# RC4ML/Legion

Hardware: AMD Instinct MI355X
Metric: sampled_edges_per_sec (higher is better)
Workload: dtype int32+f32(copy)

## Files before the change

### legion_amd/csrc/kernels_gather.hip

```cpp
#include "legion_core.h"
#include "gather_plan.h"

#include <cstdlib>
#include <cstring>
#include <type_traits>

namespace lg {

#define LG_GATHER_THREADS 256

__device__ __forceinline__ void deliver_slice(const LanePtrs& L, const DeliverParams& d, int32_t part, int32_t parts)
{
    const LG_G int32_t* nc = LG_GPTR(const int32_t, L.node_counter);
    const LG_G int32_t* ec = LG_GPTR(const int32_t, L.edge_counter);
    const LG_G int32_t* hs = LG_GPTR(const int32_t, L.hop_scratch);
    const int32_t hop_num = nc[INTRABATCH_CON * 3 - 1];
    int32_t n = nc[INTRABATCH_CON * 3 + hop_num], e = ec[INTRABATCH_CON * 3 + hop_num], b = nc[INTRABATCH_CON * 3];
    n = n < 0 ? 0 : (n > d.num_ids ? d.num_ids : n);
    e = e < 0 ? 0 : (e > d.num_ids ? d.num_ids : e);
    b = b < 0 ? 0 : (b > d.batch_cap ? d.batch_cap : b);
    const int32_t tid = threadIdx.x, nthr = blockDim.x;
    typedef int32_t v4 __attribute__((ext_vector_type(4)));
    auto copy = [&](const int32_t* src, int32_t* dst, int32_t count) {
        const int32_t per = (((count + parts - 1) / parts) + 3) & ~3;
        const int32_t lo = part * per, hi = min(lo + per, count);
        if (lo >= hi) return;
        const LG_G v4* s4 = (const LG_G v4*)(src + lo);
        LG_G v4* d4 = (LG_G v4*)(dst + lo);
        const int32_t q = (hi - lo) >> 2;
        for (int32_t i = tid; i < q; i += nthr) d4[i] = s4[i];
        for (int32_t i = lo + (q << 2) + tid; i < hi; i += nthr) LG_GPTR(int32_t, dst)[i] = LG_GPTR(const int32_t, src)[i];
    };
    copy(L.sampled_ids, d.sampled_ids, n);
    copy(L.agg_src_off, d.agg_src_off, e);
    copy(L.agg_dst_off, d.agg_dst_off, e);
    copy(L.labels, d.labels, b);
    if (part == 0 && tid < 32) {
        int32_t v = tid < 16 ? nc[tid] : ec[tid - 16];
        if (tid == 2) v = hs[HS_RANGE + 2 * hop_num];
        if (tid == 3) v = hs[HS_RANGE + 2 * hop_num + 1];
        LG_GPTR(int32_t, tid < 16 ? d.node_counter : d.edge_counter)[tid & 15] = v;
        if (d.mirror != nullptr) LG_GPTR(int32_t, d.mirror)[tid] = v;
    }
}

__global__ __launch_bounds__(256) void deliver_kernel(const LanePtrs* __restrict__ lane_p, DeliverParams d)
{
    deliver_slice(*lane_p, d, blockIdx.x, gridDim.x);
}

void launch_deliver(hipStream_t s, const LanePtrs* d_lane, const DeliverParams& d)
{
    int32_t grid = (d.num_ids / 4 + 1023) / 1024;
    if (grid > 512) grid = 512;
    if (grid < 1) grid = 1;
    deliver_kernel<<<grid, 256, 0, s>>>(d_lane, d);
    hipCheckError();
}

typedef float f32x4 __attribute__((ext_vector_type(4)));
template <typename VecT, bool TAIL> struct GatherRow {
    static_assert(std::is_same<VecT, f32x4>::value || std::is_same<VecT, float>::value, "float32 rows; bf16 rows have no TAIL pass");
    typedef float Out;
    static __device__ int32_t chunks(const GatherParams& gp) { return gp.D / (int32_t)(sizeof(VecT) / sizeof(float)); }
    static __device__ const LG_G float* row_at(const GatherParams& gp, const float* base, int64_t x) { return LG_GPTR(const float, base) + x * gp.D; }
    static __device__ VecT load(const LG_G float* p, bool, LG_G float* dst_tile, int32_t r, int32_t c, int32_t D)
    {
        if (p == nullptr) p = dst_tile + (int64_t)r * D;
        return ((const LG_G VecT*)p)[c];
    }
    static __device__ void store(const VecT& v, bool ok, LG_G float* dst_tile, int32_t r, int32_t c, int32_t D)
    {
        if (ok) __builtin_nontemporal_store(v, (LG_G VecT*)(dst_tile + (int64_t)r * D) + c);
    }
};

struct Bf16x8 {
    typedef uint32_t u4 __attribute__((ext_vector_type(4)));
    u4 w;
};
struct Bf16Copy : Bf16x8 {};
__device__ __attribute__((aligned(16))) Bf16x8 lg_gather_zero_line;
template <typename VecT, typename OutT> struct GatherRowBf16Src {
    typedef OutT Out;
    static __device__ int32_t chunks(const GatherParams& gp) { return gp.pitch / 8; }
    static __device__ const LG_G float* row_at(const GatherParams& gp, const float* base, int64_t x)
    {
        return (const LG_G float*)(LG_GPTR(const uint16_t, (const uint16_t*)base) + x * gp.pitch);
    }
    static __device__ VecT load(const LG_G float* p, bool has, LG_G Out*, int32_t, int32_t c, int32_t)
    {
        VecT v;
        v.w = has ? ((const LG_G VecT*)p)[c].w : LG_GPTR(const Bf16x8, &lg_gather_zero_line)->w;
        return v;
    }
};

template <> struct GatherRow<Bf16x8, false> : GatherRowBf16Src<Bf16x8, float> {
    static __device__ void store(const Bf16x8& v, bool ok, LG_G float* dst_tile, int32_t r, int32_t c, int32_t D)
    {
        typedef float v4u __attribute__((ext_vector_type(4), aligned(4)));
        typedef Bf16x8::u4 u4;
        const u4 lo = v.w << 16, hi = v.w & 0xFFFF0000u;
        const int32_t e0 = c * 8;
        LG_G float* d = dst_tile + (int64_t)r * D + e0;
        if (ok && e0 + 8 <= D) {
            __builtin_nontemporal_store(__builtin_bit_cast(v4u, u4{lo.x, hi.x, lo.y, hi.y}), (LG_G v4u*)d);
            __builtin_nontemporal_store(__builtin_bit_cast(v4u, u4{lo.z, hi.z, lo.w, hi.w}), (LG_G v4u*)d + 1);
        } else if (ok) {
            const uint32_t f[8] = {lo.x, hi.x, lo.y, hi.y, lo.z, hi.z, lo.w, hi.w};
#pragma unroll
            for (int k = 0; k < 8; k++)
                if (e0 + k < D) d[k] = __uint_as_float(f[k]);
        }
    }
};

__device__ __forceinline__ void gather_store_bf16(const uint32_t (&w)[4], bool ok, LG_G uint16_t* dst_tile, int32_t r, int32_t c, int32_t D)
{
    typedef uint32_t u4u __attribute__((ext_vector_type(4), aligned(4)));
    const int32_t e0 = c * 8;
    LG_G uint16_t* d = dst_tile + (int64_t)r * D + e0;
    if (ok && (D & 1) == 0) {
        if (e0 + 8 <= D) {
            __builtin_nontemporal_store(u4u{w[0], w[1], w[2], w[3]}, (LG_G u4u*)d);
        } else {
#pragma unroll
            for (int k = 0; k < 4; k++)
                if (e0 + 2 * k < D) ((LG_G uint32_t*)d)[k] = w[k];
        }
    } else if (ok) {
#pragma unroll
        for (int k = 0; k < 8; k++)
            if (e0 + k < D) d[k] = (uint16_t)(w[k >> 1] >> ((k & 1) * 16));
    }
}

template <> struct GatherRow<Bf16Copy, false> : GatherRowBf16Src<Bf16Copy, uint16_t> {
    static __device__ void store(const Bf16Copy& v, bool ok, LG_G uint16_t* dst_tile, int32_t r, int32_t c, int32_t D)
    {
        gather_store_bf16({v.w.x, v.w.y, v.w.z, v.w.w}, ok, dst_tile, r, c, D);
    }
};
__device__ __forceinline__ uint32_t gather_bf16_rne(float f)
{
    const uint32_t u = __float_as_uint(f);
    if ((u & 0x7FFFFFFFu) > 0x7F800000u) return (u >> 16) | 0x40u;
    return (u + 0x7FFFu + ((u >> 16) & 1u)) >> 16;
}

struct F32Narrow {
    typedef float v4u __attribute__((ext_vector_type(4), aligned(4)));
    v4u a, b;
};
template <> struct GatherRow<F32Narrow, false> {
    typedef uint16_t Out;
    typedef F32Narrow::v4u v4u;
    static __device__ int32_t chunks(const GatherParams& gp) { return (gp.D + 7) / 8; }
    static __device__ const LG_G float* row_at(const GatherParams& gp, const float* base, int64_t x) { return LG_GPTR(const float, base) + x * gp.D; }
    static __device__ F32Narrow load(const LG_G float* p, bool, LG_G uint16_t*, int32_t, int32_t c, int32_t D)
    {
        F32Narrow v;
        const int32_t e0 = c * 8;
        if (p == nullptr) {
            v.a = v.b = v4u{0.f, 0.f, 0.f, 0.f};
        } else if (e0 + 8 <= D) {
            v.a = ((const LG_G v4u*)(p + e0))[0];
            v.b = ((const LG_G v4u*)(p + e0))[1];
        } else {
            float f[8];
#pragma unroll
            for (int k = 0; k < 8; k++) f[k] = e0 + k < D ? p[e0 + k] : 0.f;
            v.a = v4u{f[0], f[1], f[2], f[3]};
            v.b = v4u{f[4], f[5], f[6], f[7]};
        }
        return v;
    }
    static __device__ void store(const F32Narrow& v, bool ok, LG_G uint16_t* dst_tile, int32_t r, int32_t c, int32_t D)
    {
        gather_store_bf16({gather_bf16_rne(v.a.x) | (gather_bf16_rne(v.a.y) << 16), gather_bf16_rne(v.a.z) | (gather_bf16_rne(v.a.w) << 16),
                           gather_bf16_rne(v.b.x) | (gather_bf16_rne(v.b.y) << 16), gather_bf16_rne(v.b.z) | (gather_bf16_rne(v.b.w) << 16)},
                          ok, dst_tile, r, c, D);
    }
};

#ifndef LG_GATHER_MIN_WAVES
#define LG_GATHER_MIN_WAVES 8
#endif
#ifndef LG_GATHER_TARGET_WG
#define LG_GATHER_TARGET_WG 8192
#endif

template <typename VecT, int ROWS, int UNROLL, bool TAIL, bool LASTOP>
__global__ __launch_bounds__(LG_GATHER_THREADS, LG_GATHER_MIN_WAVES) void gather_kernel(GatherParams gp, const LanePtrs* __restrict__ lanes,
                                                                   bool copy_range)
{
    typedef GatherRow<VecT, TAIL> Row;
    typedef typename Row::Out Out;
    constexpr int VEC = sizeof(VecT) / sizeof(float);
    static_assert(ROWS <= LG_GATHER_THREADS, "one resolving thread per row of a tile");
    __shared__ const LG_G float* s_ptr[2][ROWS];

    const LanePtrs& L = lanes[blockIdx.y];
    const LG_G int32_t* range = LG_GPTR(const int32_t, gp.hop >= 0 ? L.hop_scratch + HS_RANGE + 2 * gp.hop : L.node_counter);
    const LG_G int32_t* sampled_ids = LG_GPTR(const int32_t, L.sampled_ids);
    const LG_G int32_t* node_slot = (L.node_slot != nullptr && gp.node_map != nullptr) ? LG_GPTR(const int32_t, L.node_slot) : nullptr;
    LG_G int32_t* cache_search_buffer = LG_GPTR(int32_t, L.cache_search_buffer);
    int32_t off = range[0];
    int32_t rows = range[1];
    if (copy_range && blockIdx.x == 0 && threadIdx.x == 0) {
        LG_GPTR(int32_t, L.node_counter)[2] = off;
        LG_GPTR(int32_t, L.node_counter)[3] = rows;
    }
    if (gp.hop >= 0 && gp.first_hop < gp.hop) {
        const int32_t off0 = LG_GPTR(const int32_t, L.hop_scratch)[HS_RANGE + 2 * gp.first_hop];
        rows += off - off0;
        off = off0;
    }
    if (rows > gp.max_rows) rows = gp.max_rows;
    if (rows > L.feature_rows - off) {
        rows = L.feature_rows - off;
        if (blockIdx.x == 0 && threadIdx.x == 0 && L.hop_scratch != nullptr) {
            __hip_atomic_fetch_or(LG_GPTR(int32_t, L.hop_scratch) + HS_ERROR, LG_ERR_FEATURE_ROWS, __ATOMIC_RELAXED, __HIP_MEMORY_SCOPE_AGENT);
            if (L.err_flag) __hip_atomic_fetch_or(LG_GPTR(int32_t, L.err_flag), LG_ERR_FEATURE_ROWS, __ATOMIC_RELAXED, __HIP_MEMORY_SCOPE_SYSTEM);
        }
    }
    const int32_t ntiles = (rows + ROWS - 1) / ROWS;
    const int32_t step = gridDim.x;
    if (LASTOP && L.deliver != nullptr)
        deliver_slice(L, *static_cast<const DeliverParams*>(L.deliver), blockIdx.x, step);
    const int32_t tid = threadIdx.x;
    const int32_t D = gp.D;
    const int32_t C = Row::chunks(gp);
    const int32_t dr = LG_GATHER_THREADS / C;
    const int32_t dc = LG_GATHER_THREADS - dr * C;
    int32_t tile = blockIdx.x;
    if (tile >= ntiles) return;

    const bool counting = gp.stats != nullptr && gp.Kg > 1 && gp.stats[3] != 0ull;
    auto source_of = [&](int32_t id, int32_t g) -> const LG_G float* {
        const LG_G float* p = nullptr;
        if (g < 0) {
            if (id >= 0 && gp.full_table != nullptr)
                p = Row::row_at(gp, gp.full_table, (int64_t)(id < gp.total_num_nodes ? id : id % gp.total_num_nodes));
        } else if (gp.hybrid) {
            if (g < gp.hybrid_cpu_cap)
                p = Row::row_at(gp, gp.hybrid_cpu_cache, (int64_t)g);
            else
                p = Row::row_at(gp, gp.local_table, (int64_t)((g - gp.hybrid_cpu_cap) % gp.hybrid_gpu_cap));
        } else {
            int32_t didx = 0, fidx = g;
            if (gp.striped) { didx = g / gp.node_capacity; fidx = g - didx * gp.node_capacity; }
            const int64_t rank = (int64_t)fidx * gp.Kg + didx;
            const bool local_copy = gp.replica != nullptr && rank < gp.replica_rows;
            if (local_copy)
                p = Row::row_at(gp, gp.replica, rank);
            else if (didx == gp.member && gp.local_table != nullptr)
                p = Row::row_at(gp, gp.local_table, (int64_t)fidx);
            else if (gp.skip_remote)
                p = nullptr;
            else
                p = Row::row_at(gp, gp.cache_tables[didx], (int64_t)fidx);
            if (counting) {
                const unsigned long long m_rep = __ballot(local_copy), m_str = __ballot(!local_copy);
                const unsigned long long m_peer = __ballot(!local_copy && didx != gp.member);
                if ((int)(threadIdx.x & 63) == __ffsll((unsigned long long)(m_rep | m_str)) - 1) {
                    if (m_str) atomicAdd(gp.stats + 0, (unsigned long long)__popcll(m_str));
                    if (m_rep) atomicAdd(gp.stats + 1, (unsigned long long)__popcll(m_rep));
                    if (m_peer) atomicAdd(gp.stats + 2, (unsigned long long)__popcll(m_peer));
                }
            }
        }
        return p;
    };
    auto lookup = [&](int32_t id, int32_t carried) -> int32_t {
        if (carried != LG_FS_UNKNOWN) return carried;
        return (gp.node_map != nullptr && id >= 0) ? gp.node_map[id] : CACHEMISS_FLAG;
    };

    int32_t id_n = -1, fs_n = LG_FS_UNKNOWN;
    bool have_n = false;
    if (tid < ROWS) {
        const int32_t r = tile * ROWS + tid;
        if (r < rows) {
            const int32_t id = sampled_ids[off + r];
            const int32_t g = lookup(id, node_slot != nullptr ? node_slot[off + r] : LG_FS_UNKNOWN);
            cache_search_buffer[r] = g;
            s_ptr[0][tid] = source_of(id, g);
        }
        const int32_t rn = (tile + step) * ROWS + tid;
        have_n = tile + step < ntiles && rn < rows;
        if (have_n) {
            id_n = sampled_ids[off + rn];
            if (node_slot != nullptr) fs_n = node_slot[off + rn];
        }
    }
    __syncthreads();

    int buf = 0;
    for (; tile < ntiles; tile += step) {
        const int32_t r0 = tile * ROWS;
        const int32_t nr = min(ROWS, rows - r0);
        int32_t g_n = CACHEMISS_FLAG, id_nn = -1, fs_nn = LG_FS_UNKNOWN;
        bool have_nn = false;
        if (tid < ROWS) {
            if (have_n) g_n = lookup(id_n, fs_n);
            const int32_t rnn = (tile + 2 * step) * ROWS + tid;
            have_nn = tile + 2 * step < ntiles && rnn < rows;
            if (have_nn) {
                id_nn = sampled_ids[off + rnn];
                if (node_slot != nullptr) fs_nn = node_slot[off + rnn];
            }
        }

        const int32_t nchunks = nr * C;
        LG_G Out* dst_tile = LG_GPTR(Out, (Out*)L.float_features) + (int64_t)(off + r0) * D;
        int32_t q = tid;
        int32_t r = q / C;
        int32_t c = q - r * C;
        while (q < nchunks) {
            VecT v[UNROLL];
            int32_t rr[UNROLL], cc[UNROLL];
            bool ok[UNROLL];
#pragma unroll
            for (int u = 0; u < UNROLL; u++) {
                const bool in = q < nchunks;
                rr[u] = in ? r : nr - 1;
                cc[u] = in ? c : C - 1;
                const LG_G float* p = s_ptr[buf][rr[u]];
                ok[u] = in && p != nullptr;
                v[u] = Row::load(p, p != nullptr, dst_tile, rr[u], cc[u], D);
                q += LG_GATHER_THREADS;
                r += dr;
                c += dc;
                if (c >= C) { c -= C; r += 1; }
            }
#pragma unroll
            for (int u = 0; u < UNROLL; u++) Row::store(v[u], ok[u], dst_tile, rr[u], cc[u], D);
        }
        if constexpr (TAIL) {
            const int32_t tail = D - C * VEC;
            for (int32_t i = tid; i < nr * tail; i += LG_GATHER_THREADS) {
                const int32_t tr = i / tail, k = C * VEC + (i - tr * tail);
                const LG_G float* p = s_ptr[buf][tr];
                if (p != nullptr) dst_tile[(int64_t)tr * D + k] = p[k];
            }
        }
        if (tid < ROWS && have_n) {
            cache_search_buffer[(tile + step) * ROWS + tid] = g_n;
            s_ptr[buf ^ 1][tid] = source_of(id_n, g_n);
        }
        id_n = id_nn;
        fs_n = fs_nn;
        have_n = have_nn;
        __syncthreads();
        buf ^= 1;
    }
}

__global__ __launch_bounds__(256) void bulk_bucket_kernel(GatherParams gp, const LanePtrs* __restrict__ lanes, BulkLists b, const char* arena_base)
{
    const LanePtrs& L = lanes[blockIdx.y];
    const LG_G int32_t* nc = LG_GPTR(const int32_t, L.node_counter);
    const int32_t hop_num = nc[INTRABATCH_CON * 3 - 1];
    int32_t n = nc[INTRABATCH_CON * 3 + hop_num];
    if (n > L.feature_rows) n = L.feature_rows;
    if (n > gp.max_rows) n = gp.max_rows;
    const LG_G int32_t* sampled_ids = LG_GPTR(const int32_t, L.sampled_ids);
    const LG_G int32_t* node_slot = (L.node_slot != nullptr && gp.node_map != nullptr) ? LG_GPTR(const int32_t, L.node_slot) : nullptr;
    const int32_t lane = threadIdx.x & 63;
    for (int32_t r0 = (blockIdx.x * 256 + (threadIdx.x & ~63)); r0 < n; r0 += gridDim.x * 256) {
        const int32_t r = r0 + lane;
        int32_t owner = -1, fidx = 0;
        if (r < n) {
            const int32_t id = sampled_ids[r];
            int32_t g = node_slot != nullptr ? node_slot[r] : LG_FS_UNKNOWN;
            if (g == LG_FS_UNKNOWN) g = (gp.node_map != nullptr && id >= 0) ? gp.node_map[id] : CACHEMISS_FLAG;
            if (g >= 0) {
                const int32_t didx = g / gp.node_capacity;
                fidx = g - didx * gp.node_capacity;
                const int64_t rank = (int64_t)fidx * gp.Kg + didx;
                const bool local_copy = gp.replica != nullptr && rank < gp.replica_rows;
                if (!local_copy && didx != gp.member) owner = didx;
            }
        }
        for (int32_t o = 0; o < b.Kg; o++) {
            const unsigned long long m = __ballot(owner == o);
            if (m == 0ull) continue;
            unsigned long long base = 0;
            if (lane == __ffsll((long long)m) - 1) base = atomicAdd(b.cnt + o, (unsigned long long)__popcll(m));
            base = __shfl(base, __ffsll((long long)m) - 1);
            if (owner == o) {
                const int64_t at = (int64_t)base + __popcll(m & ((lane == 0) ? 0ull : (~0ull >> (64 - lane))));
                if (at < b.cap) {
                    b.fidx[(int64_t)o * b.cap + at] = fidx;
                    b.dst[(int64_t)o * b.cap + at] = (const char*)(L.float_features + (int64_t)r * gp.D) - arena_base;
                }
            }
        }
    }
}

void launch_bulk_bucket(hipStream_t s, const GatherParams& g, const LanePtrs* d_lanes, int32_t n_lanes, const BulkLists& lists,
                        const char* arena_base)
{
    if (g.D <= 0 || g.max_rows <= 0 || g.node_map == nullptr || g.Kg <= 1) return;
    GatherParams gp = g;
    if (gp.node_capacity < 1) gp.node_capacity = 1;
    int32_t gx = (g.max_rows + 255) / 256;
    while (gx > 16 && (int64_t)gx * n_lanes > 16384) gx = (gx + 1) / 2;
    bulk_bucket_kernel<<<dim3(gx, n_lanes), 256, 0, s>>>(gp, d_lanes, lists, arena_base);
    hipCheckError();
}

__global__ __launch_bounds__(256) void bulk_push_kernel(const float* __restrict__ stripe, int32_t D, const int32_t* __restrict__ fidx,
                                                       const int64_t* __restrict__ dst, const unsigned long long* __restrict__ cnt,
                                                       int64_t cap, char* __restrict__ peer_arena)
{
    typedef float v4u __attribute__((ext_vector_type(4), aligned(4)));
    int64_t n = (int64_t)cnt[0];
    if (n > cap) n = cap;
    const int32_t lane = threadIdx.x & 63;
    const int64_t wave = ((int64_t)blockIdx.x * 256 + threadIdx.x) >> 6, nwaves = ((int64_t)gridDim.x * 256) >> 6;
    const int32_t C = D / 4;
    for (int64_t i = wave; i < n; i += nwaves) {
        const LG_G float* src = LG_GPTR(const float, stripe) + (int64_t)fidx[i] * D;
        LG_G float* out = (LG_G float*)(peer_arena + dst[i]);
        for (int32_t c = lane; c < C; c += 64) ((LG_G v4u*)out)[c] = ((const LG_G v4u*)src)[c];
        for (int32_t k = C * 4 + lane; k < D; k += 64) out[k] = src[k];
    }
}

void launch_bulk_push(hipStream_t s, const float* stripe, int32_t D, const int32_t* fidx, const int64_t* dst,
                      const unsigned long long* cnt, int64_t cap, char* peer_arena)
{
    if (stripe == nullptr || D <= 0 || cap <= 0) return;
    bulk_push_kernel<<<2048, 256, 0, s>>>(stripe, D, fidx, dst, cnt, cap, peer_arena);
    hipCheckError();
}

static inline int32_t gather_grid_x(int32_t max_rows, int32_t rows_per_tile, int32_t n_lanes)
{
    const int32_t tiles = (max_rows + rows_per_tile - 1) / rows_per_tile;
    int32_t gx = (LG_GATHER_TARGET_WG + n_lanes - 1) / n_lanes;
    if (gx > tiles) gx = tiles;
    return gx < 1 ? 1 : gx;
}

template <typename VecT, GatherFormat F, int ROWS = 16>
static int32_t launch_format(hipStream_t s, int32_t rows, const GatherParams& gk, int32_t grid_rows, const LanePtrs* d_lanes, int32_t n_lanes, bool copy_range)
{
    constexpr GatherFormatInfo fi = gather_info(F);
    if constexpr ((fi.tiles & ROWS) != 0) {
        if (rows == ROWS) {
            const dim3 grid(gather_grid_x(grid_rows, ROWS, n_lanes), n_lanes);
            if (gk.last_op) gather_kernel<VecT, ROWS, fi.unroll, fi.tail, true><<<grid, LG_GATHER_THREADS, 0, s>>>(gk, d_lanes, copy_range);
            else gather_kernel<VecT, ROWS, fi.unroll, fi.tail, false><<<grid, LG_GATHER_THREADS, 0, s>>>(gk, d_lanes, copy_range);
            return (int32_t)grid.x;
        }
    }
    if constexpr (ROWS < 256) return launch_format<VecT, F, ROWS * 2>(s, rows, gk, grid_rows, d_lanes, n_lanes, copy_range);
    return 0;
}

static GatherPlan plan_of_launch(const GatherParams& gk, int32_t n_lanes, int32_t& grid_rows)
{
    grid_rows = gk.grid_rows > 0 && gk.grid_rows < gk.max_rows ? gk.grid_rows : gk.max_rows;
    return gather_plan(gk.dtype, gk.out_dtype, gk.D, gk.pitch, grid_rows, n_lanes, tuning().gather_rows_per_wg);
}

static GatherPlan launch_gather_impl(hipStream_t s, GatherParams gk, const LanePtrs* d_lanes, int32_t n_lanes, bool copy_range, int32_t* grid_x = nullptr)
{
    if (grid_x != nullptr) *grid_x = 0;
    if (gk.D <= 0 || gk.max_rows <= 0) return {GatherPlan::OK, GatherFormat::F32, 0};
    if (gk.node_capacity < 1) gk.node_capacity = 1;
    int32_t grid_rows, gx = 0;
    const GatherPlan p = plan_of_launch(gk, n_lanes, grid_rows);
    if (p.error == GatherPlan::BAD_DTYPE) printf("gather: unknown feature dtype %d or output dtype %d\n", gk.dtype, gk.out_dtype);
    if (p.error == GatherPlan::BAD_PITCH) printf("gather: bf16 rows need a pitch that is a multiple of 8 and at least D (pitch %d, D %d)\n", gk.pitch, gk.D);
    if (p.error != GatherPlan::OK) exit(EXIT_FAILURE);
    typedef GatherFormat GF;
    switch (p.format) {
        case GF::F32:       gx = launch_format<f32x4, GF::F32>(s, p.rows, gk, grid_rows, d_lanes, n_lanes, copy_range); break;
        case GF::F32Tail:   gx = launch_format<f32x4, GF::F32Tail>(s, p.rows, gk, grid_rows, d_lanes, n_lanes, copy_range); break;
        case GF::F32Scalar: gx = launch_format<float, GF::F32Scalar>(s, p.rows, gk, grid_rows, d_lanes, n_lanes, copy_range); break;
        case GF::Bf16x8:    gx = launch_format<Bf16x8, GF::Bf16x8>(s, p.rows, gk, grid_rows, d_lanes, n_lanes, copy_range); break;
        case GF::Bf16Copy:  gx = launch_format<Bf16Copy, GF::Bf16Copy>(s, p.rows, gk, grid_rows, d_lanes, n_lanes, copy_range); break;
        case GF::F32Narrow: gx = launch_format<F32Narrow, GF::F32Narrow>(s, p.rows, gk, grid_rows, d_lanes, n_lanes, copy_range); break;
    }
    hipCheckError();
    if (grid_x != nullptr) *grid_x = gx;
    return p;
}

void launch_gather(hipStream_t s, const GatherParams& g, const LanePtrs* d_lanes, int32_t n_lanes)
{
    launch_gather_impl(s, g, d_lanes, n_lanes, true);
}

int32_t launch_gather_explicit(hipStream_t s, const GatherParams& g, const int32_t* sampled_ids, const int32_t* node_slot,
                               int32_t* cache_index_out, const int32_t* range, void* dst, int32_t dst_rows, int32_t* plan_out)
{
    int32_t grid_rows, gx = 0;
    if (plan_of_launch(g, 1, grid_rows).error != GatherPlan::OK) return -1;
    static thread_local LanePtrs* d_lane = nullptr;
    if (d_lane == nullptr) HIP_CALL(hipMalloc(&d_lane, sizeof(LanePtrs)));
    LanePtrs h;
    memset(&h, 0, sizeof(h));
    h.sampled_ids = const_cast<int32_t*>(sampled_ids);
    h.node_slot = const_cast<int32_t*>(node_slot);
    h.cache_search_buffer = cache_index_out;
    h.node_counter = const_cast<int32_t*>(range);
    h.float_features = static_cast<float*>(dst);
    h.feature_rows = dst_rows;
    GatherParams ge = g;
    ge.hop = -1;
    ge.first_hop = -1;
    HIP_CALL(hipMemcpyAsync(d_lane, &h, sizeof(h), hipMemcpyHostToDevice, s));
    const GatherPlan p = launch_gather_impl(s, ge, d_lane, 1, false, &gx);
    if (plan_out != nullptr) {
        plan_out[0] = gx > 0 ? (int32_t)p.format : -1;
        plan_out[1] = gx > 0 ? p.rows : 0;
        plan_out[2] = gx;
    }
    return 0;
}

}
```

Before: 5.680 billion.

## Issue next-tile id and node-map loads unconditionally, overlapped with the feature copy

The gather loop now issues the next-next tile's id and slot loads, and the node_map lookup for the next tile, as plain branch-free loads (dummy addresses when not needed) before the feature copy. It resolves the cache slot only after the copy, so those loads overlap the row streaming. Explicit sched_barrier plus s_waitcnt calls are placed before the stores and the syncthreads to control when outstanding loads are waited on. The inner while loop becomes a do-while. This adds redundant loads and a full vmcnt wait per unroll batch, which could serialise memory traffic. The lookup() semantics are replaced with an inlined node_map read, which may not match the old lookup in every case.

```diff
diff --git a/legion_amd/csrc/kernels_gather.hip b/legion_amd/csrc/kernels_gather.hip
--- a/legion_amd/csrc/kernels_gather.hip
+++ b/legion_amd/csrc/kernels_gather.hip
@@ -184,6 +184,11 @@
     }
 };
 
+__device__ __forceinline__ void gather_wait_loads()
+{
+    __builtin_amdgcn_sched_barrier(0);
+    __builtin_amdgcn_s_waitcnt(0x0F70);
+}
 #ifndef LG_GATHER_MIN_WAVES
 #define LG_GATHER_MIN_WAVES 8
 #endif
@@ -295,22 +300,25 @@
             if (node_slot != nullptr) fs_n = node_slot[off + rn];
         }
     }
+    gather_wait_loads();
     __syncthreads();
 
+    const LG_G int32_t* row0 = sampled_ids + off;
+    const LG_G int32_t* slot_words = node_slot != nullptr ? node_slot : sampled_ids;
     int buf = 0;
     for (; tile < ntiles; tile += step) {
         const int32_t r0 = tile * ROWS;
         const int32_t nr = min(ROWS, rows - r0);
-        int32_t g_n = CACHEMISS_FLAG, id_nn = -1, fs_nn = LG_FS_UNKNOWN;
-        bool have_nn = false;
+        const int32_t rnn = (tile + 2 * step) * ROWS + tid;
+        const bool have_nn = tid < ROWS && tile + 2 * step < ntiles && rnn < rows;
+        const bool look_n = have_n && fs_n == LG_FS_UNKNOWN && gp.node_map != nullptr && id_n >= 0;
+        int32_t g_ld = CACHEMISS_FLAG, id_ld = -1, fs_ld = LG_FS_UNKNOWN;
         if (tid < ROWS) {
-            if (have_n) g_n = lookup(id_n, fs_n);
-            const int32_t rnn = (tile + 2 * step) * ROWS + tid;
-            have_nn = tile + 2 * step < ntiles && rnn < rows;
-            if (have_nn) {
-                id_nn = sampled_ids[off + rnn];
-                if (node_slot != nullptr) fs_nn = node_slot[off + rnn];
-            }
+            const int32_t at = have_nn ? off + rnn : off;
+            const LG_G int32_t* map_word = look_n ? LG_GPTR(const int32_t, gp.node_map) + id_n : row0;
+            id_ld = sampled_ids[at];
+            fs_ld = slot_words[at];
+            g_ld = *map_word;
         }
 
         const int32_t nchunks = nr * C;
@@ -318,7 +326,7 @@
         int32_t q = tid;
         int32_t r = q / C;
         int32_t c = q - r * C;
-        while (q < nchunks) {
+        do {
             VecT v[UNROLL];
             int32_t rr[UNROLL], cc[UNROLL];
             bool ok[UNROLL];
@@ -335,9 +343,10 @@
                 c += dc;
                 if (c >= C) { c -= C; r += 1; }
             }
+            gather_wait_loads();
 #pragma unroll
             for (int u = 0; u < UNROLL; u++) Row::store(v[u], ok[u], dst_tile, rr[u], cc[u], D);
-        }
+        } while (q < nchunks);
         if constexpr (TAIL) {
             const int32_t tail = D - C * VEC;
             for (int32_t i = tid; i < nr * tail; i += LG_GATHER_THREADS) {
@@ -347,11 +356,12 @@
             }
         }
         if (tid < ROWS && have_n) {
+            const int32_t g_n = fs_n != LG_FS_UNKNOWN ? fs_n : look_n ? g_ld : CACHEMISS_FLAG;
             cache_search_buffer[(tile + step) * ROWS + tid] = g_n;
             s_ptr[buf ^ 1][tid] = source_of(id_n, g_n);
         }
-        id_n = id_nn;
-        fs_n = fs_nn;
+        id_n = have_nn ? id_ld : -1;
+        fs_n = have_nn && node_slot != nullptr ? fs_ld : LG_FS_UNKNOWN;
         have_n = have_nn;
         __syncthreads();
         buf ^= 1;
```

Measured after the change: 5.687 billion, median of 2. No clear change (+0.1%).
